# Okrio/tinyrecurrentunet

Hardware: AMD Instinct MI355X
Metric: 16 kHz frames/sec (train step) (higher is better)
Workload: dtype f32; 1 GPU; config/tiny.json TRU-Net (C_in=4 incl. PCEN), 64 x 4 s 16 kHz pairs per GPU, n_fft 512 hop 128, full fp32 train step; mfma=fp32 forward, bf16x3 backward, fp32_mfma=bf16x3-bwd, frames_per_gpu=32064, global_batch=64, parallelism=dp1

## Files before the change

### tinyrecurrentunet_amd/csrc/fft.hip

```cpp
#include "common.hpp"
#include "fft_common.hpp"

namespace {

__device__ cpx* fft_lds(cpx* a, cpx* b, int n, int logn, const cpx* __restrict__ tw, bool inverse) {
    const int half = n >> 1, quarter = n >> 2;
    cpx* x = a;
    cpx* y = b;
    int ns = 1;
    int s = 0;
    if (logn & 1) {
        __syncthreads();
        for (int j = threadIdx.x; j < half; j += blockDim.x) {
            const cpx u = x[j], v = x[j + half];
            y[2 * j] = make_float2(u.x + v.x, u.y + v.y);
            y[2 * j + 1] = make_float2(u.x - v.x, u.y - v.y);
        }
        cpx* t = x; x = y; y = t;
        ns = 2;
        s = 1;
    }
    for (; s < logn; s += 2) {
        __syncthreads();
        const int tstep = quarter / ns;
// ... 13 lines not shown
            const cpx v1 = make_float2(u0.x - u2.x, u0.y - u2.y);
            const cpx v2 = make_float2(u1.x + u3.x, u1.y + u3.y);
            const cpx d = make_float2(u1.x - u3.x, u1.y - u3.y);
            const cpx v3 = inverse ? make_float2(-d.y, d.x) : make_float2(d.y, -d.x);
            const int j0 = ((j - k) << 2) + k;
            y[j0] = make_float2(v0.x + v2.x, v0.y + v2.y);
            y[j0 + ns] = make_float2(v1.x + v3.x, v1.y + v3.y);
            y[j0 + 2 * ns] = make_float2(v0.x - v2.x, v0.y - v2.y);
            y[j0 + 3 * ns] = make_float2(v1.x - v3.x, v1.y - v3.y);
        }
        cpx* t = x; x = y; y = t;
        ns <<= 2;
    }
    __syncthreads();
    return x;
}

template <int NI, bool INV>
__device__ __forceinline__ cpx* fft_lds_ni(cpx* a, cpx* b, int n, int logn, const cpx* __restrict__ tw) {
    if constexpr (NI == 2) return fft_lds_t<9, INV>(a, b, tw);
    else if constexpr (NI == 4) return fft_lds_t<10, INV>(a, b, tw);
    else if constexpr (NI == 8) return fft_lds_t<11, INV>(a, b, tw);
    else return fft_lds(a, b, n, logn, tw, INV);
}

__device__ __forceinline__ int reflect_idx(int j, int L) {
    if (j < 0) j = -j;
    if (j >= L) j = 2 * (L - 1) - j;
    return j;
}

constexpr int NF = 512;
constexpr int HOPF = 128;
constexpr int BINS = 257;

__device__ __forceinline__ float spectral_features(float re, float im, float& nm, float& sn, float& cs) {
    const float mag = sqrtf(re * re + im * im);
    const float db = 20.f * log10f(fmaxf(mag, 1e-7f)) - 25.f;
// ... 595 lines not shown
        const bool first = (fr[1] & TRUNET_ROW_FIRST) != 0;
        const int orow = fr[8];
        const float fenv = (float)fr[7];
        acc[t] = ola_add(first ? 0.f : t0, frames[(size_t)row * NF + t]);
        acc[256 + t] = ola_add(first ? 0.f : t1, frames[(size_t)row * NF + 256 + t]);
        __syncthreads();
        if (t < HOPF && orow >= 0) out[(size_t)orow * HOPF + t] = env_div(acc[t], fenv);
        t0 = acc[t + HOPF];
        t1 = (t + HOPF < 256) ? acc[256 + t + HOPF] : 0.f;
        __syncthreads();
    }
    ol[t] = t0;
    ol[256 + t] = t1;
}

template <int NI, bool YZERO>
__device__ __forceinline__ bool stft_stage_frame(cpx* sa, cpx* stw, const float* __restrict__ xb,
                                                 const float* __restrict__ yb, const float* __restrict__ win,
                                                 const cpx* __restrict__ tw, int f, int hop, int n, int L) {
    if constexpr (NI > 0) {
        float vx[NI], vy[NI], w[NI];
        cpx t[NI / 2 > 0 ? NI / 2 : 1];
#pragma unroll
        for (int it = 0; it < NI; ++it) {
            const int i = threadIdx.x + 256 * it;
            const int j = reflect_idx(f * hop + i - n / 2, L);
            vx[it] = xb[j];
            vy[it] = YZERO ? 0.f : yb[j];
            w[it] = win[i];
        }
#pragma unroll
        for (int it = 0; it < NI / 2; ++it) t[it] = tw[threadIdx.x + 256 * it];
        bool diff = false;
#pragma unroll
        for (int it = 0; it < NI; ++it) {
            const cpx z = make_float2(w[it] * vx[it], w[it] * vy[it]);
            diff |= (z.x != z.y);
            sa[threadIdx.x + 256 * it] = z;
        }
#pragma unroll
        for (int it = 0; it < NI / 2; ++it) stw[threadIdx.x + 256 * it] = t[it];
        return diff;
    } else {
        bool diff = false;
        for (int i = threadIdx.x; i < n / 2; i += 256) stw[i] = tw[i];
        for (int i = threadIdx.x; i < n; i += 256) {
            const int j = reflect_idx(f * hop + i - n / 2, L);
            const float w = win[i];
            const cpx z = make_float2(w * xb[j], YZERO ? 0.f : w * yb[j]);
            diff |= (z.x != z.y);
            sa[i] = z;
        }
        return diff;
    }
}

template <bool V> struct SameFrame { static constexpr bool value = V; };
__device__ __forceinline__ void stft_note_diff(int* wave_diff, bool diff) {
    const int any = __any(diff ? 1 : 0);
    if ((threadIdx.x & 63) == 0) wave_diff[threadIdx.x >> 6] = any;
}
__device__ __forceinline__ bool stft_same_frame(const int* wave_diff) {
    return (wave_diff[0] | wave_diff[1] | wave_diff[2] | wave_diff[3]) == 0;
}

template <int NI>
__global__ __launch_bounds__(256) void stft_loss_fwd_kernel(const float* __restrict__ x, const float* __restrict__ y,
                                                            const float* __restrict__ win, const cpx* __restrict__ tw,
                                                            float* __restrict__ partials, int L, int n, int logn, int hop,
                                                            int nframes) {
    extern __shared__ __attribute__((aligned(16))) unsigned char smraw[];
    cpx* sa = (cpx*)smraw;
    cpx* sb = sa + n;
    cpx* stw = sb + n;
    __shared__ double red[12];
    const int f = blockIdx.x, b = blockIdx.y;
    const float* xb = x + (size_t)b * L;
    const float* yb = y + (size_t)b * L;
    __shared__ int wave_diff[4];
    stft_note_diff(wave_diff, stft_stage_frame<NI, false>(sa, stw, xb, yb, win, tw, f, hop, n, L));
    const cpx* Z = fft_lds_ni<NI, false>(sa, sb, n, logn, stw);
    const bool same = stft_same_frame(wave_diff);
    float s1 = 0.f, s2 = 0.f, s3 = 0.f;
    auto bins = [&](auto same_frame) {
        for (int k = threadIdx.x; k <= n / 2; k += 256) {
            cpx X, Y;
            split_pair(Z, k, n, X, Y);
            const float xm = sqrtf(fmaxf(X.x * X.x + X.y * X.y, 1e-7f));
            const float ym = decltype(same_frame)::value ? xm : sqrtf(fmaxf(Y.x * Y.x + Y.y * Y.y, 1e-7f));
            const float d = ym - xm;
            s1 = fmaf(d, d, s1);
            s2 = fmaf(ym, ym, s2);
            s3 += fabsf(logf(ym) - logf(xm));
        }
    };
    if (same) bins(SameFrame<true>{}); else bins(SameFrame<false>{});
    s1 = wave_sum(s1); s2 = wave_sum(s2); s3 = wave_sum(s3);
    const int lane = threadIdx.x & 63, wave = threadIdx.x >> 6;
    if (lane == 0) { red[wave * 3 + 0] = (double)s1; red[wave * 3 + 1] = (double)s2; red[wave * 3 + 2] = (double)s3; }
    __syncthreads();
    if (threadIdx.x < 3) {
        float* pp = partials + ((size_t)b * nframes + f) * 3;
        pp[threadIdx.x] = (float)((red[threadIdx.x] + red[3 + threadIdx.x]) + (red[6 + threadIdx.x] + red[9 + threadIdx.x]));
    }
}

template <int NI>
__global__ __launch_bounds__(256) void stft_loss_fwdgrad_kernel(const float* __restrict__ x, const float* __restrict__ y,
                                                                const float* __restrict__ win, const cpx* __restrict__ tw,
                                                                float* __restrict__ partials, float* __restrict__ fr_sc,
                                                                float* __restrict__ fr_mag, int L, int n, int logn, int hop,
                                                                int nframes, int wl, int left) {
    extern __shared__ __attribute__((aligned(16))) unsigned char smraw[];
    cpx* sa = (cpx*)smraw;
    cpx* sb = sa + n;
    cpx* stw = sb + n;
    __shared__ double red[12];
    const int f = blockIdx.x, b = blockIdx.y;
    const float* xb = x + (size_t)b * L;
    const float* yb = y + (size_t)b * L;
    __shared__ int wave_diff[4];
    stft_note_diff(wave_diff, stft_stage_frame<NI, false>(sa, stw, xb, yb, win, tw, f, hop, n, L));
    cpx* Z = fft_lds_ni<NI, false>(sa, sb, n, logn, stw);
    const bool same = stft_same_frame(wave_diff);
    cpx* other = (Z == sa) ? sb : sa;
    float s1 = 0.f, s2 = 0.f, s3 = 0.f;
    auto bins = [&](auto same_frame) {
        for (int k = threadIdx.x; k <= n / 2; k += 256) {
            cpx X, Y;
            split_pair(Z, k, n, X, Y);
            const float px = X.x * X.x + X.y * X.y;
            const float xm = sqrtf(fmaxf(px, 1e-7f));
            const float ym = decltype(same_frame)::value ? xm : sqrtf(fmaxf(Y.x * Y.x + Y.y * Y.y, 1e-7f));
            const float d = ym - xm;
            s1 = fmaf(d, d, s1);
            s2 = fmaf(ym, ym, s2);
            const float dl = logf(xm) - logf(ym);
            s3 += fabsf(-dl);
            cpx Gs = make_float2(0.f, 0.f), Gm = Gs;
            if (px > 1e-7f) {
                const float sg = (dl > 0.f) ? 1.f : ((dl < 0.f) ? -1.f : 0.f);
                const float gs = xm - ym, gm = sg / xm;
                Gs = make_float2(gs * X.x / xm, gs * X.y / xm);
                Gm = make_float2(gm * X.x / xm, gm * X.y / xm);
            }
            if (k == 0 || k == n / 2) {
                other[k] = make_float2(Gs.x, Gm.x);
            } else {
                other[k] = make_float2(0.5f * (Gs.x - Gm.y), 0.5f * (Gs.y + Gm.x));
                other[n - k] = make_float2(0.5f * (Gs.x + Gm.y), 0.5f * (-Gs.y + Gm.x));
            }
        }
    };
    if (same) bins(SameFrame<true>{}); else bins(SameFrame<false>{});
    s1 = wave_sum(s1); s2 = wave_sum(s2); s3 = wave_sum(s3);
    const int lane = threadIdx.x & 63, wave = threadIdx.x >> 6;
    if (lane == 0) { red[wave * 3 + 0] = (double)s1; red[wave * 3 + 1] = (double)s2; red[wave * 3 + 2] = (double)s3; }
    const cpx* g = fft_lds_ni<NI, true>(other, Z, n, logn, stw);
    if (threadIdx.x < 3) {
        float* pp = partials + ((size_t)b * nframes + f) * 3;
        pp[threadIdx.x] = (float)((red[threadIdx.x] + red[3 + threadIdx.x]) + (red[6 + threadIdx.x] + red[9 + threadIdx.x]));
    }
    const size_t fo = ((size_t)b * nframes + f) * wl;
    for (int i = threadIdx.x; i < wl; i += 256) {
        const float w = win[left + i];
        const cpx v = g[left + i];
        fr_sc[fo + i] = w * v.x;
        fr_mag[fo + i] = w * v.y;
    }
}

struct LossDesc {
    const float* l1_partials; const float* parts[TRUNET_MAX_RES];
    int n_l1, nres, nrows[TRUNET_MAX_RES]; double l1_count, count[TRUNET_MAX_RES];
    float sc_lambda, mag_lambda, stft_lambda;
};
__global__ __launch_bounds__(1024) void loss_finalize_kernel(const LossDesc d, float* __restrict__ loss_out,
                                                             float* __restrict__ vals, double* __restrict__ scratch) {
    __shared__ double red[16];
    __shared__ int last;
    const int c = blockIdx.x;
    const float* src; int rows, stride;
    if (c == 0) { src = d.l1_partials; rows = d.n_l1; stride = 1; }
    else { const int i = (c - 1) / 3; src = d.parts[i] + (c - 1) % 3; rows = d.nrows[i]; stride = 3; }
// ... 76 lines not shown
                as += fs[o];
                am += fm[o];
            }
        }
        total = fmaf(vals[5 + 2 * r], as, fmaf(vals[6 + 2 * r], am, total));
    }
    g_audio[(size_t)b * L + j] = gup[0] * total;
}

template <int NI>
__global__ __launch_bounds__(256) void stft_mag_kernel(const float* __restrict__ x, const float* __restrict__ y,
                                                       const float* __restrict__ win, const cpx* __restrict__ tw,
                                                       float* __restrict__ xmag, float* __restrict__ ymag, int L, int n,
                                                       int logn, int hop, int nframes) {
    extern __shared__ __attribute__((aligned(16))) unsigned char smraw[];
    cpx* sa = (cpx*)smraw;
    cpx* sb = sa + n;
    cpx* stw = sb + n;
    const int f = blockIdx.x, b = blockIdx.y;
    const float* xb = x + (size_t)b * L;
    const float* yb = y + (size_t)b * L;
    __shared__ int wave_diff[4];
    stft_note_diff(wave_diff, stft_stage_frame<NI, false>(sa, stw, xb, yb, win, tw, f, hop, n, L));
    const cpx* Z = fft_lds_ni<NI, false>(sa, sb, n, logn, stw);
    const bool same = stft_same_frame(wave_diff);
    const size_t base = ((size_t)b * nframes + f) * (n / 2 + 1);
    auto bins = [&](auto same_frame) {
        for (int k = threadIdx.x; k <= n / 2; k += 256) {
            cpx X, Y;
            split_pair(Z, k, n, X, Y);
            const float xm = sqrtf(fmaxf(X.x * X.x + X.y * X.y, 1e-7f));
            xmag[base + k] = xm;
            if (ymag) ymag[base + k] = decltype(same_frame)::value ? xm : sqrtf(fmaxf(Y.x * Y.x + Y.y * Y.y, 1e-7f));
        }
    };
    if (same) bins(SameFrame<true>{}); else bins(SameFrame<false>{});
}

__global__ __launch_bounds__(1024) void reduce_cols_kernel(const float* __restrict__ partials, int nparts, int ncols,
                                                           float* __restrict__ out) {
    __shared__ double red[16];
    const int c = blockIdx.x;
    double s = 0.0;
    int g = threadIdx.x;
    for (; g + 3 * 1024 < nparts; g += 4 * 1024) {
        const float v0 = partials[(size_t)g * ncols + c], v1 = partials[(size_t)(g + 1024) * ncols + c];
        const float v2 = partials[(size_t)(g + 2048) * ncols + c], v3 = partials[(size_t)(g + 3072) * ncols + c];
        s += ((double)v0 + (double)v1) + ((double)v2 + (double)v3);
    }
    for (; g < nparts; g += 1024) s += (double)partials[(size_t)g * ncols + c];
#pragma unroll
    for (int o = 32; o > 0; o >>= 1) s += __shfl_xor(s, o);
    if ((threadIdx.x & 63) == 0) red[threadIdx.x >> 6] = s;
    __syncthreads();
    if (threadIdx.x == 0) {
        double t = 0.0;
#pragma unroll
        for (int k = 0; k < 16; ++k) t += red[k];
        out[c] = (float)t;
    }
}

template <bool MAG, int NI>
__global__ __launch_bounds__(256) void stft_bwd_kernel(const float* __restrict__ x, const float* __restrict__ y,
                                                       const float* __restrict__ win, const cpx* __restrict__ tw,
                                                       const float* __restrict__ coef, const float* __restrict__ gmag,
                                                       int L, int n, int logn, int hop, float* __restrict__ fr, int wl,
                                                       int left) {
    extern __shared__ __attribute__((aligned(16))) unsigned char smraw[];
    cpx* sa = (cpx*)smraw;
    cpx* sb = sa + n;
    cpx* stw = sb + n;
    const int f = blockIdx.x, b = blockIdx.y;
    const float* xb = x + (size_t)b * L;
    const float* yb = MAG ? xb : y + (size_t)b * L;
    __shared__ int wave_diff[4];
    const bool diff = stft_stage_frame<NI, MAG>(sa, stw, xb, yb, win, tw, f, hop, n, L);
    if (!MAG) stft_note_diff(wave_diff, diff);
    cpx* Z = fft_lds_ni<NI, false>(sa, sb, n, logn, stw);
    const bool same = MAG ? false : stft_same_frame(wave_diff);
    cpx* other = (Z == sa) ? sb : sa;
    const float c_sc = MAG ? 0.f : coef[0], c_mag = MAG ? 0.f : coef[1];
    const float* gm_row = MAG ? gmag + ((size_t)b * gridDim.x + f) * (n / 2 + 1) : nullptr;
    auto bins = [&](auto same_frame) {
        for (int k = threadIdx.x; k < n; k += 256) {
            cpx G = make_float2(0.f, 0.f);
            if (k <= n / 2) {
                cpx X, Y;
                split_pair(Z, k, n, X, Y);
                const float px = X.x * X.x + X.y * X.y;
                if (px > 1e-7f) {
                    const float xm = sqrtf(px);
                    float gm;
                    if (MAG) {
                        gm = gm_row[k];
                    } else {
                        const float ym = decltype(same_frame)::value ? xm : sqrtf(fmaxf(Y.x * Y.x + Y.y * Y.y, 1e-7f));
                        const float dl = logf(xm) - logf(ym);
                        const float sg = (dl > 0.f) ? 1.f : ((dl < 0.f) ? -1.f : 0.f);
                        gm = c_sc * (xm - ym) + c_mag * sg / xm;
                    }
                    G = make_float2(gm * X.x / xm, gm * X.y / xm);
                }
            }
            other[k] = G;
        }
    };
    if (same) bins(SameFrame<true>{}); else bins(SameFrame<false>{});
    const cpx* g = fft_lds_ni<NI, true>(other, Z, n, logn, stw);
    float* fo = fr + ((size_t)b * gridDim.x + f) * wl;
    for (int i = threadIdx.x; i < wl; i += 256) fo[i] = win[left + i] * g[left + i].x;
}

__global__ __launch_bounds__(256) void ola_gather_kernel(const float* __restrict__ fr, float* __restrict__ gx, int L, int n,
                                                         int hop, int nframes, int wl, int left) {
    const int b = blockIdx.y;
    const int j = blockIdx.x * 256 + threadIdx.x;
    if (j >= L) return;
    const float* fb = fr + (size_t)b * nframes * wl;
    float acc = 0.f;
#pragma unroll
    for (int which = 0; which < 3; ++which) {
        int v;
        if (which == 0) v = j;
        else if (which == 1) { if (j == 0) continue; v = -j; }
        else { if (j == L - 1) continue; v = 2 * (L - 1) - j; }
// ... 251 lines not shown
}

extern "C" int trunet_l1_grad(const float* den, const float* clean, const float* scale, float* g, int64_t n, void* stream) {
    if (!den || !clean || !scale || !g || n <= 0) return TRUNET_EINVAL;
    hipLaunchKernelGGL(l1_grad_kernel, dim3((unsigned)((n + 255) / 256)), dim3(256), 0, ST, den, clean, scale, g, n);
    return trunet_launch_status();
}

extern "C" int trunet_reduce_cols(const float* partials, int nparts, int ncols, float* out, void* stream) {
    if (!partials || !out || nparts <= 0 || ncols <= 0) return TRUNET_EINVAL;
    hipLaunchKernelGGL(reduce_cols_kernel, dim3(ncols), dim3(1024), 0, ST, partials, nparts, ncols, out);
    return trunet_launch_status();
}

constexpr int STFT_MAX_N = 2048;
static int ilog2(int n) {
    if (n < 1 || n > STFT_MAX_N) return -1;
    int l = 0;
    while ((1 << l) < n) ++l;
    return ((1 << l) == n) ? l : -1;
}

extern "C" int trunet_stft_loss_fwd(const float* x, const float* y, const float* win, const float* tw, float* partials,
                                    int B, int L, int n, int hop, void* stream) {
    const int logn = ilog2(n);
    if (!x || !y || !win || !tw || !partials || B <= 0 || logn < 3 || hop <= 0 || L <= n / 2) return TRUNET_EINVAL;
    const int nframes = 1 + L / hop;
#define FWD_(NI_) hipLaunchKernelGGL(stft_loss_fwd_kernel<NI_>, dim3(nframes, B), dim3(256), (2 * n + n / 2) * sizeof(cpx), ST, x, y, \
                                    win, (const cpx*)tw, partials, L, n, logn, hop, nframes)
    if (n == 512) FWD_(2); else if (n == 1024) FWD_(4); else if (n == 2048) FWD_(8); else FWD_(0);
#undef FWD_
    return trunet_launch_status();
}

extern "C" int trunet_stft_mag(const float* x, const float* y, const float* win, const float* tw, float* xmag, float* ymag,
                               int B, int L, int n, int hop, void* stream) {
    const int logn = ilog2(n);
    if (!x || !win || !tw || !xmag || B <= 0 || logn < 3 || hop <= 0 || L <= n / 2) return TRUNET_EINVAL;
    const int nframes = 1 + L / hop;
#define MAG_(NI_) hipLaunchKernelGGL(stft_mag_kernel<NI_>, dim3(nframes, B), dim3(256), (2 * n + n / 2) * sizeof(cpx), ST, x, y ? y : x, \
                                    win, (const cpx*)tw, xmag, y ? ymag : nullptr, L, n, logn, hop, nframes)
    if (n == 512) MAG_(2); else if (n == 1024) MAG_(4); else if (n == 2048) MAG_(8); else MAG_(0);
#undef MAG_
    return trunet_launch_status();
}

extern "C" int trunet_stft_loss_bwd_gather(const float* x, const float* y, const float* win, const float* tw,
                                           const float* coef, float* frames, float* gx, int B, int L, int n, int hop,
                                           int win_length, void* stream) {
    const int logn = ilog2(n);
    if (!x || !y || !win || !tw || !coef || !frames || !gx || B <= 0 || logn < 3 || hop <= 0 || L <= n / 2 ||
        win_length <= 0 || win_length > n)
        return TRUNET_EINVAL;
    const int nframes = 1 + L / hop;
    const int left = (n - win_length) / 2;
#define BWD_(NI_) hipLaunchKernelGGL((stft_bwd_kernel<false, NI_>), dim3(nframes, B), dim3(256), (2 * n + n / 2) * sizeof(cpx), ST, x, y, \
                                    win, (const cpx*)tw, coef, (const float*)nullptr, L, n, logn, hop, frames, win_length, left)
    if (n == 512) BWD_(2); else if (n == 1024) BWD_(4); else if (n == 2048) BWD_(8); else BWD_(0);
#undef BWD_
    hipLaunchKernelGGL(ola_gather_kernel, dim3((L + 255) / 256, B), dim3(256), 0, ST, frames, gx, L, n, hop, nframes,
                       win_length, left);
    return trunet_launch_status();
}

extern "C" int trunet_stream_features(float* ring, const float* chunk, float* pcen_M, float* feat, const float* tw512, int S,
                                      int C, int first, float eps, float s, float alpha, float delta, float r, void* stream) {
    if (!ring || !feat || !tw512 || S <= 0 || (C != 3 && C != 4) || (C == 4 && !pcen_M)) return TRUNET_EINVAL;
    hipLaunchKernelGGL(stream_features_kernel, dim3((S + 1) / 2), dim3(256), 0, ST, ring, chunk, pcen_M, feat, (const cpx*)tw512,
                       S, C, first, eps, s, alpha, delta, r, powf(delta, r));
    return trunet_launch_status();
}

// ... 62 lines not shown
        (n_out > 0 && !out) || slots <= 0)
        return TRUNET_EINVAL;
    hipLaunchKernelGGL(stream_feed_ola_kernel, dim3(n_sess), dim3(256), 0, ST, frames, ola, out, rows, sess, seq, n_rows, n_out,
                       slots);
    return trunet_launch_status();
}

extern "C" int trunet_stft_loss_fwdgrad(const float* x, const float* y, const float* win, const float* tw, float* partials,
                                        float* fr_sc, float* fr_mag, int B, int L, int n, int hop, int win_length, void* stream) {
    const int logn = ilog2(n);
    if (!x || !y || !win || !tw || !partials || !fr_sc || !fr_mag || B <= 0 || logn < 3 || hop <= 0 || L <= n / 2 ||
        win_length <= 0 || win_length > n)
        return TRUNET_EINVAL;
    const int nframes = 1 + L / hop;
    const int left = (n - win_length) / 2;
#define FG_(NI_) hipLaunchKernelGGL(stft_loss_fwdgrad_kernel<NI_>, dim3(nframes, B), dim3(256), (2 * n + n / 2) * sizeof(cpx), ST, x, y, \
                                   win, (const cpx*)tw, partials, fr_sc, fr_mag, L, n, logn, hop, nframes, win_length, left)
    if (n == 512) FG_(2); else if (n == 1024) FG_(4); else if (n == 2048) FG_(8); else FG_(0);
#undef FG_
    return trunet_launch_status();
}

extern "C" size_t trunet_loss_scratch_bytes(void) { return (1 + 3 * TRUNET_MAX_RES + 1) * sizeof(double); }

extern "C" int trunet_loss_finalize(const trunet_loss_args* a, float* loss_out, float* vals, void* scratch, void* stream) {
    if (!a || !loss_out || !vals || !scratch || !a->l1_partials || a->n_l1 <= 0 || !(a->l1_count > 0) || a->nres < 0 ||
        a->nres > TRUNET_MAX_RES)
        return TRUNET_EINVAL;
    LossDesc d;
    d.l1_partials = a->l1_partials; d.n_l1 = a->n_l1; d.nres = a->nres; d.l1_count = a->l1_count;
    d.sc_lambda = a->sc_lambda; d.mag_lambda = a->mag_lambda; d.stft_lambda = a->stft_lambda;
// ... 19 lines not shown
        d.wl[i] = a->win_length[i]; d.nframes[i] = 1 + L / a->hop[i];
    }
    hipLaunchKernelGGL(loss_grad_gather_kernel, dim3((L + 255) / 256, B), dim3(256), 0, ST, d, audio, clean, vals, g_loss,
                       g_audio, L);
    return trunet_launch_status();
}

extern "C" int trunet_stft_mag_bwd(const float* x, const float* win, const float* tw, const float* gmag, float* frames,
                                   float* gx, int B, int L, int n, int hop, int win_length, void* stream) {
    const int logn = ilog2(n);
    if (!x || !win || !tw || !gmag || !frames || !gx || B <= 0 || logn < 3 || hop <= 0 || L <= n / 2 ||
        win_length <= 0 || win_length > n)
        return TRUNET_EINVAL;
    const int nframes = 1 + L / hop;
    const int left = (n - win_length) / 2;
#define BWD_(NI_) hipLaunchKernelGGL((stft_bwd_kernel<true, NI_>), dim3(nframes, B), dim3(256), (2 * n + n / 2) * sizeof(cpx), ST, x, x, \
                                    win, (const cpx*)tw, (const float*)nullptr, gmag, L, n, logn, hop, frames, win_length, left)
    if (n == 512) BWD_(2); else if (n == 1024) BWD_(4); else if (n == 2048) BWD_(8); else BWD_(0);
#undef BWD_
    hipLaunchKernelGGL(ola_gather_kernel, dim3((L + 255) / 256, B), dim3(256), 0, ST, frames, gx, L, n, hop, nframes,
                       win_length, left);
    return trunet_launch_status();
}

extern "C" int trunet_phm_bwd(const float* mix_ri, const float* est_ri, const float* g_out, float* g_mix_ri, float* g_est_ri,
                              int64_t n, float beta, void* stream) {
    if (!mix_ri || !est_ri || !g_out || (!g_mix_ri && !g_est_ri) || n <= 0) return TRUNET_EINVAL;
    hipLaunchKernelGGL(phm_bwd_kernel, dim3((unsigned)((n + 255) / 256)), dim3(256), 0, ST, (const float2*)mix_ri,
                       (const float2*)est_ri, g_out, (float2*)g_mix_ri, (float2*)g_est_ri, n, beta);
    return trunet_launch_status();
}

// ... 49 lines not shown
```

### tinyrecurrentunet_amd/csrc/fft_common.hpp

```cpp
#pragma once
#include "common.hpp"

namespace {

typedef float2 cpx;

__device__ __forceinline__ cpx cmul(cpx a, cpx b) { return make_float2(a.x * b.x - a.y * b.y, a.x * b.y + a.y * b.x); }
__device__ __forceinline__ cpx cconj(cpx a) { return make_float2(a.x, -a.y); }

template <int LOGN, bool INV>
__device__ __forceinline__ cpx* fft_lds_t(cpx* a, cpx* b, const cpx* __restrict__ tw) {
    constexpr int n = 1 << LOGN, half = n >> 1, quarter = n >> 2;
    cpx* x = a;
    cpx* y = b;
    if constexpr (LOGN & 1) {
        __syncthreads();
#pragma unroll
        for (int it = 0; it < (half + 255) / 256; ++it) {
            const int j = threadIdx.x + 256 * it;
            if (half >= 256 || j < half) {
                const cpx u = x[j], v = x[j + half];
                y[2 * j] = make_float2(u.x + v.x, u.y + v.y);
                y[2 * j + 1] = make_float2(u.x - v.x, u.y - v.y);
            }
// ... 26 lines not shown
                const cpx d = make_float2(u1.x - u3.x, u1.y - u3.y);
                const cpx v3 = INV ? make_float2(-d.y, d.x) : make_float2(d.y, -d.x);
                const int j0 = ((j - k) << 2) + k;
                y[j0] = make_float2(v0.x + v2.x, v0.y + v2.y);
                y[j0 + ns] = make_float2(v1.x + v3.x, v1.y + v3.y);
                y[j0 + 2 * ns] = make_float2(v0.x - v2.x, v0.y - v2.y);
                y[j0 + 3 * ns] = make_float2(v1.x - v3.x, v1.y - v3.y);
            }
        }
        cpx* t = x; x = y; y = t;
    }
    __syncthreads();
    return x;
}

__device__ __forceinline__ void split_pair(const cpx* Z, int k, int n, cpx& A, cpx& B) {
    const cpx zk = Z[k];
    const cpx zn = cconj(Z[(n - k) & (n - 1)]);
    A = make_float2(0.5f * (zk.x + zn.x), 0.5f * (zk.y + zn.y));
    B = make_float2(0.5f * (zk.y - zn.y), -0.5f * (zk.x - zn.x));
}

}
```

Measured before the change: 760,900 frames/s.

## Compute one STFT frame per wavefront with register-resident mixed-radix FFT

Replaces the block-per-frame radix-4 LDS FFT with a per-wavefront, register-based mixed-radix (8/16) FFT that processes four frames per 256-thread block. Each wave keeps its frame in registers, exchanges data through a private LDS slice, and uses wave-level barriers instead of block-wide __syncthreads. Interior frames load contiguously without reflection. This cuts block barriers and LDS round trips per butterfly stage, at the cost of higher register pressure and more complex indexing.

```diff
diff --git a/tinyrecurrentunet_amd/csrc/fft.hip b/tinyrecurrentunet_amd/csrc/fft.hip
--- a/tinyrecurrentunet_amd/csrc/fft.hip
+++ b/tinyrecurrentunet_amd/csrc/fft.hip
@@ -51,14 +51,6 @@
     }
     __syncthreads();
     return x;
-}
-
-template <int NI, bool INV>
-__device__ __forceinline__ cpx* fft_lds_ni(cpx* a, cpx* b, int n, int logn, const cpx* __restrict__ tw) {
-    if constexpr (NI == 2) return fft_lds_t<9, INV>(a, b, tw);
-    else if constexpr (NI == 4) return fft_lds_t<10, INV>(a, b, tw);
-    else if constexpr (NI == 8) return fft_lds_t<11, INV>(a, b, tw);
-    else return fft_lds(a, b, n, logn, tw, INV);
 }
 
 __device__ __forceinline__ int reflect_idx(int j, int L) {
@@ -684,44 +676,87 @@
     ol[256 + t] = t1;
 }
 
-template <int NI, bool YZERO>
+template <bool YZERO>
 __device__ __forceinline__ bool stft_stage_frame(cpx* sa, cpx* stw, const float* __restrict__ xb,
                                                  const float* __restrict__ yb, const float* __restrict__ win,
                                                  const cpx* __restrict__ tw, int f, int hop, int n, int L) {
-    if constexpr (NI > 0) {
-        float vx[NI], vy[NI], w[NI];
-        cpx t[NI / 2 > 0 ? NI / 2 : 1];
-#pragma unroll
-        for (int it = 0; it < NI; ++it) {
-            const int i = threadIdx.x + 256 * it;
-            const int j = reflect_idx(f * hop + i - n / 2, L);
-            vx[it] = xb[j];
-            vy[it] = YZERO ? 0.f : yb[j];
-            w[it] = win[i];
-        }
-#pragma unroll
-        for (int it = 0; it < NI / 2; ++it) t[it] = tw[threadIdx.x + 256 * it];
-        bool diff = false;
-#pragma unroll
-        for (int it = 0; it < NI; ++it) {
-            const cpx z = make_float2(w[it] * vx[it], w[it] * vy[it]);
-            diff |= (z.x != z.y);
-            sa[threadIdx.x + 256 * it] = z;
-        }
-#pragma unroll
-        for (int it = 0; it < NI / 2; ++it) stw[threadIdx.x + 256 * it] = t[it];
-        return diff;
+    bool diff = false;
+    for (int i = threadIdx.x; i < n / 2; i += 256) stw[i] = tw[i];
+    for (int i = threadIdx.x; i < n; i += 256) {
+        const int j = reflect_idx(f * hop + i - n / 2, L);
+        const float w = win[i];
+        const cpx z = make_float2(w * xb[j], YZERO ? 0.f : w * yb[j]);
+        diff |= (z.x != z.y);
+        sa[i] = z;
+    }
+    return diff;
+}
+
+template <int NI, bool YZERO>
+__device__ __forceinline__ bool stft_stage_regs(cpx (&v)[StftPlan<NI>::P], cpx* stw, const float* __restrict__ xb,
+                                                const float* __restrict__ yb, const float* __restrict__ win,
+                                                const cpx* __restrict__ tw, int f, int nframes, int hop, int L) {
+    typedef StftPlan<NI> S;
+    const int lane = threadIdx.x & 63;
+    cpx t[NI / 2];
+#pragma unroll
+    for (int it = 0; it < NI / 2; ++it) t[it] = tw[threadIdx.x + 256 * it];
+    float vx[S::P], vy[S::P], w[S::P];
+    const int s0 = f * hop - S::n / 2;
+    if (NI < 8 && f < nframes && s0 >= 0 && s0 + S::n <= L) {
+        const float* xp = xb + s0 + lane;
+        const float* yp = yb + s0 + lane;
+#pragma unroll
+        for (int c = 0; c < S::P; ++c) {
+            vx[c] = xp[64 * c];
+            vy[c] = YZERO ? 0.f : yp[64 * c];
+            w[c] = win[lane + 64 * c];
+        }
+    } else if (f < nframes) {
+#pragma unroll
+        for (int c = 0; c < S::P; ++c) {
+            const int i = lane + 64 * c;
+            const int j = reflect_idx(s0 + i, L);
+            vx[c] = xb[j];
+            vy[c] = YZERO ? 0.f : yb[j];
+            w[c] = win[i];
+        }
     } else {
-        bool diff = false;
-        for (int i = threadIdx.x; i < n / 2; i += 256) stw[i] = tw[i];
-        for (int i = threadIdx.x; i < n; i += 256) {
-            const int j = reflect_idx(f * hop + i - n / 2, L);
-            const float w = win[i];
-            const cpx z = make_float2(w * xb[j], YZERO ? 0.f : w * yb[j]);
-            diff |= (z.x != z.y);
-            sa[i] = z;
-        }
-        return diff;
+#pragma unroll
+        for (int c = 0; c < S::P; ++c) vx[c] = vy[c] = w[c] = 0.f;
+    }
+#pragma unroll
+    for (int it = 0; it < NI / 2; ++it) stw[threadIdx.x + 256 * it] = t[it];
+    bool diff = false;
+#pragma unroll
+    for (int c = 0; c < S::P; ++c) {
+        v[c] = make_float2(w[c] * vx[c], w[c] * vy[c]);
+        diff |= (v[c].x != v[c].y);
+    }
+    __syncthreads();
+    return diff;
+}
+
+template <int NI>
+__device__ __forceinline__ cpx* stft_wave_buf(cpx* stw) {
+    return stw + StftPlan<NI>::half + (threadIdx.x >> 6) * StftPlan<NI>::FRAME;
+}
+
+template <int NI, bool TWO>
+__device__ __forceinline__ void stft_write_frame(const cpx (&v)[StftPlan<NI>::P], const float* __restrict__ win,
+                                                 float* __restrict__ fa, float* __restrict__ fb, size_t fo, int wl,
+                                                 int left) {
+    const int i0 = (threadIdx.x & 63) - left;
+    const float* wp = win + left + i0;
+    float* pa = fa + fo + i0;
+    float* pb = TWO ? fb + fo + i0 : nullptr;
+#pragma unroll
+    for (int c = 0; c < StftPlan<NI>::P; ++c) {
+        if ((unsigned)(i0 + 64 * c) < (unsigned)wl) {
+            const float w = wp[64 * c];
+            pa[64 * c] = w * v[c].x;
+            if (TWO) pb[64 * c] = w * v[c].y;
+        }
     }
 }
 
@@ -732,6 +767,78 @@
 }
 __device__ __forceinline__ bool stft_same_frame(const int* wave_diff) {
     return (wave_diff[0] | wave_diff[1] | wave_diff[2] | wave_diff[3]) == 0;
+}
+
+struct StftFrame {
+    cpx* Z; cpx* other; cpx* stw;
+    int f, n, k0, kstep;
+    bool live, same;
+};
+
+template <int NI, bool YZERO, bool NOTE_DIFF>
+__device__ __forceinline__ StftFrame stft_forward(cpx (&v)[NI > 0 ? 4 * NI : 1], unsigned char* smraw,
+                                                  const float* __restrict__ xb, const float* __restrict__ yb,
+                                                  const float* __restrict__ win, const cpx* __restrict__ tw, int n, int logn,
+                                                  int hop, int L, int nframes) {
+    StftFrame F;
+    if constexpr (NI > 0) {
+        typedef StftPlan<NI> S;
+        const int lane = threadIdx.x & 63;
+        F.stw = (cpx*)smraw;
+        F.f = blockIdx.x * S::FPB + (threadIdx.x >> 6);
+        F.n = S::n; F.k0 = lane; F.kstep = 64;
+        F.live = F.f < nframes;
+        const bool diff = stft_stage_regs<NI, YZERO>(v, F.stw, xb, yb, win, tw, F.f, nframes, hop, L);
+        F.same = NOTE_DIFF && !__any(diff ? 1 : 0);
+        F.Z = F.other = stft_wave_buf<NI>(F.stw);
+        if (F.live) stft_fft_fwd<NI>(v, F.Z, F.stw, lane);
+    } else {
+        cpx* sa = (cpx*)smraw;
+        cpx* sb = sa + n;
+        F.stw = sb + n;
+        __shared__ int wave_diff[4];
+        F.f = blockIdx.x; F.n = n; F.k0 = threadIdx.x; F.kstep = 256;
+        F.live = true;
+        const bool diff = stft_stage_frame<YZERO>(sa, F.stw, xb, yb, win, tw, F.f, hop, n, L);
+        if (NOTE_DIFF) stft_note_diff(wave_diff, diff);
+        F.Z = fft_lds(sa, sb, n, logn, F.stw, false);
+        F.same = NOTE_DIFF && stft_same_frame(wave_diff);
+        F.other = (F.Z == sa) ? sb : sa;
+    }
+    return F;
+}
+
+template <int NI>
+__device__ __forceinline__ void stft_write_sums(float s1, float s2, float s3, float* __restrict__ pp) {
+    s1 = wave_sum(s1); s2 = wave_sum(s2); s3 = wave_sum(s3);
+    const int lane = threadIdx.x & 63, wave = threadIdx.x >> 6;
+    if constexpr (NI > 0) {
+        if (lane == 0) { pp[0] = s1; pp[1] = s2; pp[2] = s3; }
+    } else {
+        __shared__ double red[12];
+        if (lane == 0) { red[wave * 3 + 0] = (double)s1; red[wave * 3 + 1] = (double)s2; red[wave * 3 + 2] = (double)s3; }
+        __syncthreads();
+        if (threadIdx.x < 3)
+            pp[threadIdx.x] = (float)((red[threadIdx.x] + red[3 + threadIdx.x]) + (red[6 + threadIdx.x] + red[9 + threadIdx.x]));
+    }
+}
+
+template <int NI, bool TWO>
+__device__ __forceinline__ void stft_inverse_write(cpx (&v)[NI > 0 ? 4 * NI : 1], const StftFrame& F, int logn,
+                                                   const float* __restrict__ win, float* __restrict__ fa,
+                                                   float* __restrict__ fb, size_t fo, int wl, int left) {
+    if constexpr (NI > 0) {
+        stft_fft_inv<NI>(v, F.other, F.stw, threadIdx.x & 63);
+        stft_write_frame<NI, TWO>(v, win, fa, fb, fo, wl, left);
+    } else {
+        const cpx* g = fft_lds(F.other, F.Z, F.n, logn, F.stw, true);
+        for (int i = threadIdx.x; i < wl; i += 256) {
+            const float w = win[left + i];
+            const cpx t = g[left + i];
+            fa[fo + i] = w * t.x;
+            if (TWO) fb[fo + i] = w * t.y;
+        }
+    }
 }
 
 template <int NI>
@@ -740,22 +847,18 @@
                                                             float* __restrict__ partials, int L, int n, int logn, int hop,
                                                             int nframes) {
     extern __shared__ __attribute__((aligned(16))) unsigned char smraw[];
-    cpx* sa = (cpx*)smraw;
-    cpx* sb = sa + n;
-    cpx* stw = sb + n;
-    __shared__ double red[12];
-    const int f = blockIdx.x, b = blockIdx.y;
+    const int b = blockIdx.y;
     const float* xb = x + (size_t)b * L;
     const float* yb = y + (size_t)b * L;
-    __shared__ int wave_diff[4];
-    stft_note_diff(wave_diff, stft_stage_frame<NI, false>(sa, stw, xb, yb, win, tw, f, hop, n, L));
-    const cpx* Z = fft_lds_ni<NI, false>(sa, sb, n, logn, stw);
-    const bool same = stft_same_frame(wave_diff);
+    cpx v[NI > 0 ? 4 * NI : 1];
+    const StftFrame F = stft_forward<NI, false, true>(v, smraw, xb, yb, win, tw, n, logn, hop, L, nframes);
+    if (!F.live) return;
+    const cpx* Z = F.Z;
     float s1 = 0.f, s2 = 0.f, s3 = 0.f;
     auto bins = [&](auto same_frame) {
-        for (int k = threadIdx.x; k <= n / 2; k += 256) {
+        for (int k = F.k0; k <= F.n / 2; k += F.kstep) {
             cpx X, Y;
-            split_pair(Z, k, n, X, Y);
+            split_pair(Z, k, F.n, X, Y);
             const float xm = sqrtf(fmaxf(X.x * X.x + X.y * X.y, 1e-7f));
             const float ym = decltype(same_frame)::value ? xm : sqrtf(fmaxf(Y.x * Y.x + Y.y * Y.y, 1e-7f));
             const float d = ym - xm;
@@ -764,15 +867,8 @@
             s3 += fabsf(logf(ym) - logf(xm));
         }
     };
-    if (same) bins(SameFrame<true>{}); else bins(SameFrame<false>{});
-    s1 = wave_sum(s1); s2 = wave_sum(s2); s3 = wave_sum(s3);
-    const int lane = threadIdx.x & 63, wave = threadIdx.x >> 6;
-    if (lane == 0) { red[wave * 3 + 0] = (double)s1; red[wave * 3 + 1] = (double)s2; red[wave * 3 + 2] = (double)s3; }
-    __syncthreads();
-    if (threadIdx.x < 3) {
-        float* pp = partials + ((size_t)b * nframes + f) * 3;
-        pp[threadIdx.x] = (float)((red[threadIdx.x] + red[3 + threadIdx.x]) + (red[6 + threadIdx.x] + red[9 + threadIdx.x]));
-    }
+    if (F.same) bins(SameFrame<true>{}); else bins(SameFrame<false>{});
+    stft_write_sums<NI>(s1, s2, s3, partials + ((size_t)b * nframes + F.f) * 3);
 }
 
 template <int NI>
@@ -782,23 +878,19 @@
                                                                 float* __restrict__ fr_mag, int L, int n, int logn, int hop,
                                                                 int nframes, int wl, int left) {
     extern __shared__ __attribute__((aligned(16))) unsigned char smraw[];
-    cpx* sa = (cpx*)smraw;
-    cpx* sb = sa + n;
-    cpx* stw = sb + n;
-    __shared__ double red[12];
-    const int f = blockIdx.x, b = blockIdx.y;
+    const int b = blockIdx.y;
     const float* xb = x + (size_t)b * L;
     const float* yb = y + (size_t)b * L;
-    __shared__ int wave_diff[4];
-    stft_note_diff(wave_diff, stft_stage_frame<NI, false>(sa, stw, xb, yb, win, tw, f, hop, n, L));
-    cpx* Z = fft_lds_ni<NI, false>(sa, sb, n, logn, stw);
-    const bool same = stft_same_frame(wave_diff);
-    cpx* other = (Z == sa) ? sb : sa;
+    cpx v[NI > 0 ? 4 * NI : 1];
+    const StftFrame F = stft_forward<NI, false, true>(v, smraw, xb, yb, win, tw, n, logn, hop, L, nframes);
+    if (!F.live) return;
+    const cpx* Z = F.Z;
+    cpx* other = F.other;
     float s1 = 0.f, s2 = 0.f, s3 = 0.f;
     auto bins = [&](auto same_frame) {
-        for (int k = threadIdx.x; k <= n / 2; k += 256) {
+        for (int k = F.k0; k <= F.n / 2; k += F.kstep) {
             cpx X, Y;
-            split_pair(Z, k, n, X, Y);
+            split_pair(Z, k, F.n, X, Y);
             const float px = X.x * X.x + X.y * X.y;
             const float xm = sqrtf(fmaxf(px, 1e-7f));
             const float ym = decltype(same_frame)::value ? xm : sqrtf(fmaxf(Y.x * Y.x + Y.y * Y.y, 1e-7f));
@@ -814,30 +906,17 @@
                 Gs = make_float2(gs * X.x / xm, gs * X.y / xm);
                 Gm = make_float2(gm * X.x / xm, gm * X.y / xm);
             }
-            if (k == 0 || k == n / 2) {
+            if (k == 0 || k == F.n / 2) {
                 other[k] = make_float2(Gs.x, Gm.x);
             } else {
                 other[k] = make_float2(0.5f * (Gs.x - Gm.y), 0.5f * (Gs.y + Gm.x));
-                other[n - k] = make_float2(0.5f * (Gs.x + Gm.y), 0.5f * (-Gs.y + Gm.x));
+                other[F.n - k] = make_float2(0.5f * (Gs.x + Gm.y), 0.5f * (-Gs.y + Gm.x));
             }
         }
     };
-    if (same) bins(SameFrame<true>{}); else bins(SameFrame<false>{});
-    s1 = wave_sum(s1); s2 = wave_sum(s2); s3 = wave_sum(s3);
-    const int lane = threadIdx.x & 63, wave = threadIdx.x >> 6;
-    if (lane == 0) { red[wave * 3 + 0] = (double)s1; red[wave * 3 + 1] = (double)s2; red[wave * 3 + 2] = (double)s3; }
-    const cpx* g = fft_lds_ni<NI, true>(other, Z, n, logn, stw);
-    if (threadIdx.x < 3) {
-        float* pp = partials + ((size_t)b * nframes + f) * 3;
-        pp[threadIdx.x] = (float)((red[threadIdx.x] + red[3 + threadIdx.x]) + (red[6 + threadIdx.x] + red[9 + threadIdx.x]));
-    }
-    const size_t fo = ((size_t)b * nframes + f) * wl;
-    for (int i = threadIdx.x; i < wl; i += 256) {
-        const float w = win[left + i];
-        const cpx v = g[left + i];
-        fr_sc[fo + i] = w * v.x;
-        fr_mag[fo + i] = w * v.y;
-    }
+    if (F.same) bins(SameFrame<true>{}); else bins(SameFrame<false>{});
+    stft_write_sums<NI>(s1, s2, s3, partials + ((size_t)b * nframes + F.f) * 3);
+    stft_inverse_write<NI, true>(v, F, logn, win, fr_sc, fr_mag, ((size_t)b * nframes + F.f) * wl, wl, left);
 }
 
 struct LossDesc {
@@ -944,27 +1023,24 @@
                                                        float* __restrict__ xmag, float* __restrict__ ymag, int L, int n,
                                                        int logn, int hop, int nframes) {
     extern __shared__ __attribute__((aligned(16))) unsigned char smraw[];
-    cpx* sa = (cpx*)smraw;
-    cpx* sb = sa + n;
-    cpx* stw = sb + n;
-    const int f = blockIdx.x, b = blockIdx.y;
+    const int b = blockIdx.y;
     const float* xb = x + (size_t)b * L;
     const float* yb = y + (size_t)b * L;
-    __shared__ int wave_diff[4];
-    stft_note_diff(wave_diff, stft_stage_frame<NI, false>(sa, stw, xb, yb, win, tw, f, hop, n, L));
-    const cpx* Z = fft_lds_ni<NI, false>(sa, sb, n, logn, stw);
-    const bool same = stft_same_frame(wave_diff);
-    const size_t base = ((size_t)b * nframes + f) * (n / 2 + 1);
+    cpx v[NI > 0 ? 4 * NI : 1];
+    const StftFrame F = stft_forward<NI, false, true>(v, smraw, xb, yb, win, tw, n, logn, hop, L, nframes);
+    if (!F.live) return;
+    const cpx* Z = F.Z;
+    const size_t base = ((size_t)b * nframes + F.f) * (F.n / 2 + 1);
     auto bins = [&](auto same_frame) {
-        for (int k = threadIdx.x; k <= n / 2; k += 256) {
+        for (int k = F.k0; k <= F.n / 2; k += F.kstep) {
             cpx X, Y;
-            split_pair(Z, k, n, X, Y);
+            split_pair(Z, k, F.n, X, Y);
             const float xm = sqrtf(fmaxf(X.x * X.x + X.y * X.y, 1e-7f));
             xmag[base + k] = xm;
             if (ymag) ymag[base + k] = decltype(same_frame)::value ? xm : sqrtf(fmaxf(Y.x * Y.x + Y.y * Y.y, 1e-7f));
         }
     };
-    if (same) bins(SameFrame<true>{}); else bins(SameFrame<false>{});
+    if (F.same) bins(SameFrame<true>{}); else bins(SameFrame<false>{});
 }
 
 __global__ __launch_bounds__(1024) void reduce_cols_kernel(const float* __restrict__ partials, int nparts, int ncols,
@@ -995,51 +1071,44 @@
 __global__ __launch_bounds__(256) void stft_bwd_kernel(const float* __restrict__ x, const float* __restrict__ y,
                                                        const float* __restrict__ win, const cpx* __restrict__ tw,
                                                        const float* __restrict__ coef, const float* __restrict__ gmag,
-                                                       int L, int n, int logn, int hop, float* __restrict__ fr, int wl,
-                                                       int left) {
+                                                       int L, int n, int logn, int hop, int nframes, float* __restrict__ fr,
+                                                       int wl, int left) {
     extern __shared__ __attribute__((aligned(16))) unsigned char smraw[];
-    cpx* sa = (cpx*)smraw;
-    cpx* sb = sa + n;
-    cpx* stw = sb + n;
-    const int f = blockIdx.x, b = blockIdx.y;
+    const int b = blockIdx.y;
     const float* xb = x + (size_t)b * L;
     const float* yb = MAG ? xb : y + (size_t)b * L;
-    __shared__ int wave_diff[4];
-    const bool diff = stft_stage_frame<NI, MAG>(sa, stw, xb, yb, win, tw, f, hop, n, L);
-    if (!MAG) stft_note_diff(wave_diff, diff);
-    cpx* Z = fft_lds_ni<NI, false>(sa, sb, n, logn, stw);
-    const bool same = MAG ? false : stft_same_frame(wave_diff);
-    cpx* other = (Z == sa) ? sb : sa;
+    cpx v[NI > 0 ? 4 * NI : 1];
+    const StftFrame F = stft_forward<NI, MAG, !MAG>(v, smraw, xb, yb, win, tw, n, logn, hop, L, nframes);
+    if (!F.live) return;
+    const cpx* Z = F.Z;
+    cpx* other = F.other;
     const float c_sc = MAG ? 0.f : coef[0], c_mag = MAG ? 0.f : coef[1];
-    const float* gm_row = MAG ? gmag + ((size_t)b * gridDim.x + f) * (n / 2 + 1) : nullptr;
+    const float* gm_row = MAG ? gmag + ((size_t)b * nframes + F.f) * (F.n / 2 + 1) : nullptr;
     auto bins = [&](auto same_frame) {
-        for (int k = threadIdx.x; k < n; k += 256) {
+        for (int k = F.k0; k <= F.n / 2; k += F.kstep) {
             cpx G = make_float2(0.f, 0.f);
-            if (k <= n / 2) {
-                cpx X, Y;
-                split_pair(Z, k, n, X, Y);
-                const float px = X.x * X.x + X.y * X.y;
-                if (px > 1e-7f) {
-                    const float xm = sqrtf(px);
-                    float gm;
-                    if (MAG) {
-                        gm = gm_row[k];
-                    } else {
-                        const float ym = decltype(same_frame)::value ? xm : sqrtf(fmaxf(Y.x * Y.x + Y.y * Y.y, 1e-7f));
-                        const float dl = logf(xm) - logf(ym);
-                        const float sg = (dl > 0.f) ? 1.f : ((dl < 0.f) ? -1.f : 0.f);
-                        gm = c_sc * (xm - ym) + c_mag * sg / xm;
-                    }
-                    G = make_float2(gm * X.x / xm, gm * X.y / xm);
+            cpx X, Y;
+            split_pair(Z, k, F.n, X, Y);
+            const float px = X.x * X.x + X.y * X.y;
+            if (px > 1e-7f) {
+                const float xm = sqrtf(px);
+                float gm;
+                if (MAG) {
+                    gm = gm_row[k];
+                } else {
+                    const float ym = decltype(same_frame)::value ? xm : sqrtf(fmaxf(Y.x * Y.x + Y.y * Y.y, 1e-7f));
+                    const float dl = logf(xm) - logf(ym);
+                    const float sg = (dl > 0.f) ? 1.f : ((dl < 0.f) ? -1.f : 0.f);
+                    gm = c_sc * (xm - ym) + c_mag * sg / xm;
                 }
+                G = make_float2(gm * X.x / xm, gm * X.y / xm);
             }
             other[k] = G;
+            if (k > 0 && k < F.n / 2) other[F.n - k] = make_float2(0.f, 0.f);
         }
     };
-    if (same) bins(SameFrame<true>{}); else bins(SameFrame<false>{});
-    const cpx* g = fft_lds_ni<NI, true>(other, Z, n, logn, stw);
-    float* fo = fr + ((size_t)b * gridDim.x + f) * wl;
-    for (int i = threadIdx.x; i < wl; i += 256) fo[i] = win[left + i] * g[left + i].x;
+    if (F.same) bins(SameFrame<true>{}); else bins(SameFrame<false>{});
+    stft_inverse_write<NI, false>(v, F, logn, win, fr, nullptr, ((size_t)b * nframes + F.f) * wl, wl, left);
 }
 
 __global__ __launch_bounds__(256) void ola_gather_kernel(const float* __restrict__ fr, float* __restrict__ gx, int L, int n,
@@ -1321,6 +1390,22 @@
 }
 
 constexpr int STFT_MAX_N = 2048;
+
+template <int NI> constexpr size_t stft_lds_bytes(int n) {
+    if constexpr (NI > 0) return StftPlan<NI>::LDS_BYTES; else return (size_t)(2 * n + n / 2) * sizeof(cpx);
+}
+template <int NI> constexpr int stft_grid_x(int nframes) {
+    if constexpr (NI > 0) return (nframes + StftPlan<NI>::FPB - 1) / StftPlan<NI>::FPB; else return nframes;
+}
+#define STFT_LAUNCH_(KERN_, NI_, ...)                                                                                         \
+    do {                                                                                                                      \
+        auto kern_ = KERN_;                                                                                                   \
+        const size_t lds_ = stft_lds_bytes<NI_>(n);                                                                           \
+        if (lds_ > 64 * 1024 &&                                                                                               \
+            hipFuncSetAttribute((const void*)kern_, hipFuncAttributeMaxDynamicSharedMemorySize, (int)lds_) != hipSuccess)     \
+            return TRUNET_ELAUNCH;                                                                                            \
+        hipLaunchKernelGGL(kern_, dim3(stft_grid_x<NI_>(nframes), B), dim3(256), lds_, ST, __VA_ARGS__);                      \
+    } while (0)
 static int ilog2(int n) {
     if (n < 1 || n > STFT_MAX_N) return -1;
     int l = 0;
@@ -1333,7 +1418,7 @@
     const int logn = ilog2(n);
     if (!x || !y || !win || !tw || !partials || B <= 0 || logn < 3 || hop <= 0 || L <= n / 2) return TRUNET_EINVAL;
     const int nframes = 1 + L / hop;
-#define FWD_(NI_) hipLaunchKernelGGL(stft_loss_fwd_kernel<NI_>, dim3(nframes, B), dim3(256), (2 * n + n / 2) * sizeof(cpx), ST, x, y, \
+#define FWD_(NI_) STFT_LAUNCH_(stft_loss_fwd_kernel<NI_>, NI_, x, y, \
                                     win, (const cpx*)tw, partials, L, n, logn, hop, nframes)
     if (n == 512) FWD_(2); else if (n == 1024) FWD_(4); else if (n == 2048) FWD_(8); else FWD_(0);
 #undef FWD_
@@ -1345,7 +1430,7 @@
     const int logn = ilog2(n);
     if (!x || !win || !tw || !xmag || B <= 0 || logn < 3 || hop <= 0 || L <= n / 2) return TRUNET_EINVAL;
     const int nframes = 1 + L / hop;
-#define MAG_(NI_) hipLaunchKernelGGL(stft_mag_kernel<NI_>, dim3(nframes, B), dim3(256), (2 * n + n / 2) * sizeof(cpx), ST, x, y ? y : x, \
+#define MAG_(NI_) STFT_LAUNCH_(stft_mag_kernel<NI_>, NI_, x, y ? y : x, \
                                     win, (const cpx*)tw, xmag, y ? ymag : nullptr, L, n, logn, hop, nframes)
     if (n == 512) MAG_(2); else if (n == 1024) MAG_(4); else if (n == 2048) MAG_(8); else MAG_(0);
 #undef MAG_
@@ -1361,8 +1446,8 @@
         return TRUNET_EINVAL;
     const int nframes = 1 + L / hop;
     const int left = (n - win_length) / 2;
-#define BWD_(NI_) hipLaunchKernelGGL((stft_bwd_kernel<false, NI_>), dim3(nframes, B), dim3(256), (2 * n + n / 2) * sizeof(cpx), ST, x, y, \
-                                    win, (const cpx*)tw, coef, (const float*)nullptr, L, n, logn, hop, frames, win_length, left)
+#define BWD_(NI_) STFT_LAUNCH_((stft_bwd_kernel<false, NI_>), NI_, x, y, \
+                                    win, (const cpx*)tw, coef, (const float*)nullptr, L, n, logn, hop, nframes, frames, win_length, left)
     if (n == 512) BWD_(2); else if (n == 1024) BWD_(4); else if (n == 2048) BWD_(8); else BWD_(0);
 #undef BWD_
     hipLaunchKernelGGL(ola_gather_kernel, dim3((L + 255) / 256, B), dim3(256), 0, ST, frames, gx, L, n, hop, nframes,
@@ -1455,7 +1540,7 @@
         return TRUNET_EINVAL;
     const int nframes = 1 + L / hop;
     const int left = (n - win_length) / 2;
-#define FG_(NI_) hipLaunchKernelGGL(stft_loss_fwdgrad_kernel<NI_>, dim3(nframes, B), dim3(256), (2 * n + n / 2) * sizeof(cpx), ST, x, y, \
+#define FG_(NI_) STFT_LAUNCH_(stft_loss_fwdgrad_kernel<NI_>, NI_, x, y, \
                                    win, (const cpx*)tw, partials, fr_sc, fr_mag, L, n, logn, hop, nframes, win_length, left)
     if (n == 512) FG_(2); else if (n == 1024) FG_(4); else if (n == 2048) FG_(8); else FG_(0);
 #undef FG_
@@ -1505,8 +1590,8 @@
         return TRUNET_EINVAL;
     const int nframes = 1 + L / hop;
     const int left = (n - win_length) / 2;
-#define BWD_(NI_) hipLaunchKernelGGL((stft_bwd_kernel<true, NI_>), dim3(nframes, B), dim3(256), (2 * n + n / 2) * sizeof(cpx), ST, x, x, \
-                                    win, (const cpx*)tw, (const float*)nullptr, gmag, L, n, logn, hop, frames, win_length, left)
+#define BWD_(NI_) STFT_LAUNCH_((stft_bwd_kernel<true, NI_>), NI_, x, x, \
+                                    win, (const cpx*)tw, (const float*)nullptr, gmag, L, n, logn, hop, nframes, frames, win_length, left)
     if (n == 512) BWD_(2); else if (n == 1024) BWD_(4); else if (n == 2048) BWD_(8); else BWD_(0);
 #undef BWD_
     hipLaunchKernelGGL(ola_gather_kernel, dim3((L + 255) / 256, B), dim3(256), 0, ST, frames, gx, L, n, hop, nframes,
diff --git a/tinyrecurrentunet_amd/csrc/fft_common.hpp b/tinyrecurrentunet_amd/csrc/fft_common.hpp
--- a/tinyrecurrentunet_amd/csrc/fft_common.hpp
+++ b/tinyrecurrentunet_amd/csrc/fft_common.hpp
@@ -64,6 +64,181 @@
     return x;
 }
 
+template <int NI>
+struct StftPlan {
+    static constexpr int n = 256 * NI, half = n / 2, P = n / 64;
+    static constexpr int LOGH = NI == 2 ? 8 : (NI == 4 ? 9 : 10);
+    static constexpr int R0 = NI == 2 ? 8 : 16, R1 = NI == 8 ? 16 : 8;
+    static constexpr int U0 = P / R0, U1 = P / R1, U2 = P / 8;
+    static constexpr int M = n / R0, G = n / 8;
+    static constexpr int AS = 64 + 4 / U0, GS = G + 8;
+    static constexpr int FRAME = P * AS > 8 * GS ? P * AS : 8 * GS;
+    static constexpr int FPB = 4;
+    static constexpr size_t LDS_BYTES = (size_t)(half + FPB * FRAME) * sizeof(cpx);
+    static_assert(NI == 2 || NI == 4 || NI == 8, "n = 512, 1024 or 2048");
+    static_assert(R0 * R1 * 8 == n && U0 * R0 == P && U1 * R1 == P && U1 * 8 == R0 && FRAME >= n, "digit factors");
+};
+
+__device__ __forceinline__ cpx cadd(cpx a, cpx b) { return make_float2(a.x + b.x, a.y + b.y); }
+__device__ __forceinline__ cpx csub(cpx a, cpx b) { return make_float2(a.x - b.x, a.y - b.y); }
+template <bool INV>
+__device__ __forceinline__ cpx cmulc(cpx a, float wr, float wi) {
+    return cmul(a, make_float2(wr, INV ? wi : -wi));
+}
+template <bool INV>
+__device__ __forceinline__ cpx cmulj(cpx a) { return INV ? make_float2(-a.y, a.x) : make_float2(a.y, -a.x); }
+
+template <bool INV>
+__device__ __forceinline__ void dft4(cpx& a0, cpx& a1, cpx& a2, cpx& a3) {
+    const cpx t0 = cadd(a0, a2), t1 = csub(a0, a2), t2 = cadd(a1, a3), t3 = cmulj<INV>(csub(a1, a3));
+    a0 = cadd(t0, t2); a1 = cadd(t1, t3); a2 = csub(t0, t2); a3 = csub(t1, t3);
+}
+template <bool INV>
+__device__ __forceinline__ void dft8(cpx* a) {
+    constexpr float H = 0.70710678118654752f;
+    cpx s0 = cadd(a[0], a[4]), s1 = cadd(a[1], a[5]), s2 = cadd(a[2], a[6]), s3 = cadd(a[3], a[7]);
+    cpx d0 = csub(a[0], a[4]), d1 = cmulc<INV>(csub(a[1], a[5]), H, H), d2 = cmulj<INV>(csub(a[2], a[6])),
+        d3 = cmulc<INV>(csub(a[3], a[7]), -H, H);
+    dft4<INV>(s0, s1, s2, s3);
+    dft4<INV>(d0, d1, d2, d3);
+    a[0] = s0; a[1] = d0; a[2] = s1; a[3] = d1; a[4] = s2; a[5] = d2; a[6] = s3; a[7] = d3;
+}
+template <bool INV>
+__device__ __forceinline__ void dft16(cpx* a) {
+    constexpr float H = 0.70710678118654752f, C1 = 0.92387953251128674f, S1 = 0.38268343236508977f;
+    cpx s[8], d[8];
+#pragma unroll
+    for (int i = 0; i < 8; ++i) { s[i] = cadd(a[i], a[i + 8]); d[i] = csub(a[i], a[i + 8]); }
+    d[1] = cmulc<INV>(d[1], C1, S1);
+    d[2] = cmulc<INV>(d[2], H, H);
+    d[3] = cmulc<INV>(d[3], S1, C1);
+    d[4] = cmulj<INV>(d[4]);
+    d[5] = cmulc<INV>(d[5], -S1, C1);
+    d[6] = cmulc<INV>(d[6], -H, H);
+    d[7] = cmulc<INV>(d[7], -C1, S1);
+    dft8<INV>(s);
+    dft8<INV>(d);
+#pragma unroll
+    for (int i = 0; i < 8; ++i) { a[2 * i] = s[i]; a[2 * i + 1] = d[i]; }
+}
+template <int R, bool INV>
+__device__ __forceinline__ void dft_r(cpx* a) {
+    if constexpr (R == 8) dft8<INV>(a); else dft16<INV>(a);
+}
+
+template <int NI, bool INV>
+__device__ __forceinline__ cpx stft_tw(const cpx* stw, int t) {
+    typedef StftPlan<NI> S;
+    const cpx w = stw[t & (S::half - 1)];
+    const unsigned neg = (unsigned)(t & S::half) << (31 - S::LOGH);
+    return make_float2(__uint_as_float(__float_as_uint(w.x) ^ neg),
+                       __uint_as_float(__float_as_uint(w.y) ^ neg ^ (INV ? 0x80000000u : 0u)));
+}
+
+__device__ __forceinline__ void stft_wave_sync() {
+    __builtin_amdgcn_fence(__ATOMIC_ACQ_REL, "wavefront");
+    __builtin_amdgcn_wave_barrier();
+}
+
+template <int NI>
+__device__ __forceinline__ int stft_apos(int p) { return (p >> 6) * StftPlan<NI>::AS + (p & 63); }
+
+template <int NI>
+__device__ __forceinline__ void stft_fft_fwd(cpx (&v)[StftPlan<NI>::P], cpx* fb, const cpx* stw, int lane) {
+    typedef StftPlan<NI> S;
+#pragma unroll
+    for (int u = 0; u < S::U0; ++u) {
+        cpx a[S::R0];
+#pragma unroll
+        for (int m = 0; m < S::R0; ++m) a[m] = v[u + S::U0 * m];
+        dft_r<S::R0, false>(a);
+        const int j = lane + 64 * u;
+        fb[u * S::AS + lane] = a[0];
+#pragma unroll
+        for (int q = 1; q < S::R0; ++q) fb[(u + S::U0 * q) * S::AS + lane] = cmul(a[q], stft_tw<NI, false>(stw, j * q));
+    }
+    stft_wave_sync();
+    const int j1 = lane >> 3, q0l = lane & 7;
+#pragma unroll
+    for (int u = 0; u < S::U1; ++u)
+#pragma unroll
+        for (int m = 0; m < S::R1; ++m) v[u * S::R1 + m] = fb[stft_apos<NI>((q0l + 8 * u) * S::M + j1 + 8 * m)];
+    stft_wave_sync();
+#pragma unroll
+    for (int u = 0; u < S::U1; ++u) {
+        cpx* a = &v[u * S::R1];
+        dft_r<S::R1, false>(a);
+        const int o = j1 * S::GS + q0l + 8 * u;
+        fb[o] = a[0];
+#pragma unroll
+        for (int q = 1; q < S::R1; ++q) fb[o + S::R0 * q] = cmul(a[q], stft_tw<NI, false>(stw, S::R0 * j1 * q));
+    }
+    stft_wave_sync();
+#pragma unroll
+    for (int u = 0; u < S::U2; ++u)
+#pragma unroll
+        for (int m = 0; m < 8; ++m) v[u * 8 + m] = fb[m * S::GS + lane + 64 * u];
+    stft_wave_sync();
+#pragma unroll
+    for (int u = 0; u < S::U2; ++u) {
+        dft8<false>(&v[u * 8]);
+#pragma unroll
+        for (int q = 0; q < 8; ++q) fb[lane + 64 * u + S::G * q] = v[u * 8 + q];
+    }
+    stft_wave_sync();
+}
+
+template <int NI>
+__device__ __forceinline__ void stft_fft_inv(cpx (&v)[StftPlan<NI>::P], cpx* fb, const cpx* stw, int lane) {
+    typedef StftPlan<NI> S;
+    stft_wave_sync();
+#pragma unroll
+    for (int u = 0; u < S::U2; ++u)
+#pragma unroll
+        for (int q = 0; q < 8; ++q) v[u * 8 + q] = fb[lane + 64 * u + S::G * q];
+    stft_wave_sync();
+#pragma unroll
+    for (int u = 0; u < S::U2; ++u) {
+        dft8<true>(&v[u * 8]);
+#pragma unroll
+        for (int m = 0; m < 8; ++m) fb[m * S::GS + lane + 64 * u] = v[u * 8 + m];
+    }
+    stft_wave_sync();
+    const int j1 = lane >> 3, q0l = lane & 7;
+#pragma unroll
+    for (int u = 0; u < S::U1; ++u) {
+        const int o = j1 * S::GS + q0l + 8 * u;
+        v[u * S::R1] = fb[o];
+#pragma unroll
+        for (int q = 1; q < S::R1; ++q) v[u * S::R1 + q] = fb[o + S::R0 * q];
+    }
+    stft_wave_sync();
+#pragma unroll
+    for (int u = 0; u < S::U1; ++u) {
+        cpx* a = &v[u * S::R1];
+#pragma unroll
+        for (int q = 1; q < S::R1; ++q) a[q] = cmul(a[q], stft_tw<NI, true>(stw, S::R0 * j1 * q));
+        dft_r<S::R1, true>(a);
+#pragma unroll
+        for (int m = 0; m < S::R1; ++m) fb[stft_apos<NI>((q0l + 8 * u) * S::M + j1 + 8 * m)] = a[m];
+    }
+    stft_wave_sync();
+    cpx r[S::P];
+#pragma unroll
+    for (int c = 0; c < S::P; ++c) r[c] = fb[c * S::AS + lane];
+#pragma unroll
+    for (int u = 0; u < S::U0; ++u) {
+        cpx a[S::R0];
+        const int j = lane + 64 * u;
+        a[0] = r[u];
+#pragma unroll
+        for (int q = 1; q < S::R0; ++q) a[q] = cmul(r[u + S::U0 * q], stft_tw<NI, true>(stw, j * q));
+        dft_r<S::R0, true>(a);
+#pragma unroll
+        for (int m = 0; m < S::R0; ++m) v[u + S::U0 * m] = a[m];
+    }
+}
+
 __device__ __forceinline__ void split_pair(const cpx* Z, int k, int n, cpx& A, cpx& B) {
     const cpx zk = Z[k];
     const cpx zn = cconj(Z[(n - k) & (n - 1)]);
```

After: 763,700 frames/s, median of 6. No clear change (+0.4%).
